# lebrice/blurred-GAN

Measured on AMD Instinct MI355X. Metric: images/sec (G+D+GP step), higher is better.
Workload: dtype f32; 1 GPU; celeba64 64x64x3 batch 256/GPU, blur sigma 5.0 (31 taps), D-step+GP+G-step+Adam; global_batch=256, parallelism=dp1

## Files before the change

blurred-gan_amd/csrc/conv_rows.hip:

```cpp
#include "conv_common.h"
#include <algorithm>
#include <cstdlib>
#include <cstring>
#include <type_traits>

namespace {

typedef float floatx4 __attribute__((ext_vector_type(4)));

struct RowParams {
  const float* A;
  const float* Wt;
  float* C;
  int B, Hi, Wi, Ck, Ho, Wo, N;
  int pt, pl, flip;
  int R, strips;
  int wpr, ipw;
  int epi_mode;
  const float* bias;
  const float* ref;
  const unsigned char* keep;
  size_t keep_elems;
  float alpha, scale;
};
// ... 82 lines not shown
  int e_src[NE][NTERM];
  unsigned e_dst[NE];
  float e_bias[NE], e_mul[NE];
  int e_n[NE];
  if (tid < 2 * S) pbuf[(size_t)tid * PS + PIXW * 17] = 0.f;
  {
    const int per_img = p.Wo * N;
#pragma unroll
    for (int q = 0; q < NE; ++q) {
      const int e = tid + q * NTH;
      const int im = e / per_img, rem = e - im * per_img;
      const int x = rem / N, n = rem - x * N;
      const bool ok = e < p.ipw * per_img && im < nimg;
      e_dst[q] = ok ? (unsigned)(((im * p.Ho * p.Wo + x) * N + n) * 4) : kOob;
      e_n[q] = n;
      e_bias[q] = ok && p.bias ? p.bias[n] : 0.f;
      e_mul[q] = ok && p.epi_mode == BG_EPI_AFFINE_LRELU ? p.ref[n] : 0.f;
#pragma unroll
      for (int i = 0; i < NTERM; ++i) {
        const int kw = (x + p.pl) % S + i * S;
        const int num = x + p.pl - kw, ix = num / S;
        e_src[q][i] = (ok && kw < K && num >= 0 && ix < p.Wi) ? (im * p.Wi + ix) * 17 + kw * N + n : PIXW * 17;
      }
    }
  }
  const size_t out0 = img0 * p.Ho * p.Wo * N;
  auto pwrite = [&](const floatx4& pacc, int slot) {
    float* pb = pbuf + (size_t)slot * PS;
#pragma unroll
    for (int rr = 0; rr < 4; ++rr) pb[((size_t)img * p.Wi + 16 * t + 4 * kq + rr) * 17 + li] = pacc[rr];
  };
  auto pstore = [&](int slot, int y, bool live) {
    const float* pb = pbuf + (size_t)slot * PS;
    float v[NE];
#pragma unroll
    for (int q = 0; q < NE; ++q) {
      v[q] = pb[e_src[q][0]];
#pragma unroll
      for (int i = 1; i < NTERM; ++i) v[q] += pb[e_src[q][i]];
    }
    const unsigned add = live ? (unsigned)(y * p.Wo * N * 4) : 0u, force = live ? 0u : kOob;
#pragma unroll
    for (int q = 0; q < NE; ++q) {
      const unsigned off = (e_dst[q] + add) | force;
      float o;
      if (EP == 0) {
        o = v[q] + e_bias[q];
      } else if (EP == 1) {
        o = tanh_branchless(v[q] + e_bias[q]);
      } else {
        const bool mine = (off & kOob) == 0;
        o = mine ? bg::apply_epilogue_pre(p, v[q], out0 + (off >> 2), e_bias[q], e_mul[q]) : 0.f;
      }
      __builtin_amdgcn_raw_buffer_store_b32(__builtin_bit_cast(unsigned, o), rsC, off, 0, 0);
    }
  };

  float4 g0[NQ], g1[NQ], g2[NQ], g3[NQ];
  gload(0, g0);
  gload(1, g1);
  gload(2, g2);
  gload(3, g3);
  lstore(0, g0);
  gload(4, g0);
#pragma unroll
  for (int i = 0; i < 4 * NE * S; ++i) __builtin_amdgcn_raw_buffer_store_b32(0u, rsC, kOob + 4u * i, 0, 0);
  int y_prev = 0;
  bool have_prev = false;
  auto flush_prev = [&](int prev_par) {
#pragma unroll
    for (int kh = 0; kh < S; ++kh) {
      const int y = y_prev + kh;
      pstore(prev_par * S + kh, y, have_prev & (y >= y0) & (y < y1));
    }
  };
  auto trip = [&](int r, auto parity, float4 (&g)[NQ]) {
    constexpr int cur = decltype(parity)::value;
    __syncthreads();
    float a[KS];
#pragma unroll
    for (int ks = 0; ks < KS; ++ks) a[ks] = afrag[(size_t)cur * PIXW * AS + 4 * ks];
#pragma unroll
    for (int ks = 0; ks < KS; ++ks)
#pragma unroll
      for (int kh = 0; kh < K; ++kh) acc[kh] = __builtin_amdgcn_mfma_f32_16x16x4f32(a[ks], bw[kh][ks], acc[kh], 0, 0, 0);
    flush_prev(cur ^ 1);
    lstore(cur ^ 1, g);
    gload(r + 5, g);
#pragma unroll
    for (int kh = 0; kh < S; ++kh) pwrite(acc[kh], cur * S + kh);
    y_prev = (iy_lo + r) * S - p.pt;
    have_prev = true;
#pragma unroll
    for (int i = 0; i < K; ++i) acc[i] = i + S < K ? acc[i + S] : floatx4{0.f, 0.f, 0.f, 0.f};
  };
  int r = 0;
  for (; r + 4 <= nrows; r += 4) {
    trip(r, std::integral_constant<int, 0>{}, g1);
    trip(r + 1, std::integral_constant<int, 1>{}, g2);
    trip(r + 2, std::integral_constant<int, 0>{}, g3);
    trip(r + 3, std::integral_constant<int, 1>{}, g0);
  }
  int last_par = 1;
  if (r < nrows) {
    trip(r, std::integral_constant<int, 0>{}, g1);
    last_par = 0;
    if (r + 1 < nrows) {
      trip(r + 1, std::integral_constant<int, 1>{}, g2);
      last_par = 1;
      if (r + 2 < nrows) {
        trip(r + 2, std::integral_constant<int, 0>{}, g3);
        last_par = 0;
      }
    }
  }
  __syncthreads();
  if (last_par == 0) flush_prev(0); else flush_prev(1);
}

template <int K, int S>
int launch_rows(const RowParams& p, dim3 grid, size_t lds, hipStream_t s) {
  const bool wide = p.Wi == 128;
  const int ep = p.epi_mode == BG_EPI_NONE ? 0 : p.epi_mode == BG_EPI_TANH ? 1 : 2;
#define BG_RS2(KSv, EPv) do { if (wide) bg::launch((conv_rows_scatter_kernel<KSv, K, S, 128, EPv>), grid, dim3(512), lds, s, p); \
                              else bg::launch((conv_rows_scatter_kernel<KSv, K, S, 64, EPv>), grid, dim3(256), lds, s, p); } while (0)
#define BG_RS(KSv) do { if (ep == 0) BG_RS2(KSv, 0); else if (ep == 1) BG_RS2(KSv, 1); else BG_RS2(KSv, 2); } while (0)
  switch (p.Ck) {
    case 16: BG_RS(4); return 1;
    case 32: BG_RS(8); return 1;
    case 64: BG_RS(16); return 1;
    default: return 0;
  }
#undef BG_RS
#undef BG_RS2
}

constexpr int kRgHalo = 16;

struct RowGParams {
  const float* A;
  const float* Wt;
  float* C;
  int B, Hi, Wi, Ct, Ho, Wo, N;
  int s, pt, pl, flip;
  int R, strips;
  int epi_mode;
  const float* bias;
  const float* ref;
  const unsigned char* keep;
  size_t keep_elems;
  float alpha, scale;
};

template <int TG, int NT, int K, bool MASK>
__global__ __launch_bounds__(256) void conv_rows_gather_kernel(const RowGParams p) {
  extern __shared__ __attribute__((aligned(16))) float xl[];
  const int tid = threadIdx.x, lane = tid & 63, wave = tid >> 6;
  const int li = lane & 15, kq = lane >> 4;
  const int Ct = p.Ct, N = 16 * NT, st = p.s;
  const int RS = p.Wi * Ct + 2 * kRgHalo;
  const int strip = blockIdx.x % p.strips, b = blockIdx.x / p.strips;
  const int oy0 = strip * p.R, rows = min(p.R, p.Ho - oy0);
  const int nrows_in = (rows - 1) * st + K;

  float bw[K][4][NT];
#pragma unroll
  for (int ks = 0; ks < 4; ++ks) {
    const int i = 4 * ks + kq, kw = i / Ct, ci = i - kw * Ct;
#pragma unroll
    for (int kh = 0; kh < K; ++kh) {
      const int tap = p.flip ? (K - 1 - kh) * K + (K - 1 - kw) : kh * K + kw;
#pragma unroll
      for (int nt = 0; nt < NT; ++nt) bw[kh][ks][nt] = i < K * Ct ? p.Wt[((size_t)tap * N + nt * 16 + li) * Ct + ci] : 0.f;
    }
  }
  const int RL = p.Wi * Ct;
  if ((RL & 3) == 0) {
    const int q4 = RS / 4;
    bg::stage_rows_f4<4>(xl, nrows_in, q4, RS, tid, [&](int r, int c4) -> const float* {
      const int iy = oy0 * st - p.pt + r, e = c4 * 4 - kRgHalo;
      return ((unsigned)iy < (unsigned)p.Hi && (unsigned)e < (unsigned)RL) ? p.A + ((size_t)b * p.Hi + iy) * RL + e : nullptr;
    });
  } else {
    for (int idx = tid; idx < nrows_in * RS; idx += 256) {
      const int r = idx / RS, c = idx - r * RS;
      const int iy = oy0 * st - p.pt + r, e = c - kRgHalo;
      float v = 0.f;
      if ((unsigned)iy < (unsigned)p.Hi && (unsigned)e < (unsigned)RL) v = p.A[((size_t)b * p.Hi + iy) * RL + e];
      xl[idx] = v;
    }
  }
  __syncthreads();

  float e_bias[NT], e_mul[NT];
#pragma unroll
  for (int nt = 0; nt < NT; ++nt) {
    e_bias[nt] = p.bias ? p.bias[nt * 16 + li] : 0.f;
    e_mul[nt] = p.epi_mode == BG_EPI_AFFINE_LRELU ? p.ref[nt * 16 + li] : 1.f;
  }
  const int groups = p.Wo / (16 * TG);
  const int nunits = rows * groups;
  for (int u = wave; u < nunits; u += 4) {
    const int r = u / groups, g = u - r * groups;
    const int oy = oy0 + r, ox0 = g * 16 * TG;
    floatx4 acc[TG][NT];
#pragma unroll
    for (int tg = 0; tg < TG; ++tg)
#pragma unroll
      for (int nt = 0; nt < NT; ++nt) acc[tg][nt] = floatx4{0.f, 0.f, 0.f, 0.f};
    const float* abase = xl + (size_t)(r * st) * RS + kRgHalo + ((ox0 + li) * st - p.pl) * Ct + kq;
#pragma unroll
    for (int kh = 0; kh < K; ++kh) {
      float a[TG][4];
#pragma unroll
      for (int tg = 0; tg < TG; ++tg)
#pragma unroll
        for (int ks = 0; ks < 4; ++ks) a[tg][ks] = abase[(size_t)kh * RS + tg * 16 * st * Ct + 4 * ks];
#pragma unroll
      for (int ks = 0; ks < 4; ++ks)
#pragma unroll
        for (int tg = 0; tg < TG; ++tg)
#pragma unroll
          for (int nt = 0; nt < NT; ++nt) acc[tg][nt] = __builtin_amdgcn_mfma_f32_16x16x4f32(a[tg][ks], bw[kh][ks][nt], acc[tg][nt], 0, 0, 0);
    }
    constexpr bool mask_epi = MASK;
#pragma unroll
    for (int tg = 0; tg < TG; ++tg) {
      const size_t pix0 = ((size_t)b * p.Ho + oy) * p.Wo + ox0 + 16 * tg + 4 * kq;
      unsigned char e_keep[4][NT];
      if (mask_epi) {
#pragma unroll
        for (int rr = 0; rr < 4; ++rr)
#pragma unroll
          for (int nt = 0; nt < NT; ++nt) {
            const size_t idx = (pix0 + rr) * N + nt * 16 + li;
            e_keep[rr][nt] = p.keep[(p.keep_elems == 0 || idx < p.keep_elems) ? idx : 0];
          }
      }
#pragma unroll
      for (int rr = 0; rr < 4; ++rr)
#pragma unroll
        for (int nt = 0; nt < NT; ++nt) {
          const size_t idx = (pix0 + rr) * N + nt * 16 + li;
          if (mask_epi) {
            float v = acc[tg][nt][rr] + e_bias[nt];
            v = v > 0.f ? v : p.alpha * v;
            if (p.keep_elems == 0 || idx < p.keep_elems) v = e_keep[rr][nt] ? v * p.scale : 0.f;
            p.C[idx] = v;
          } else {
            p.C[idx] = bg::apply_epilogue_pre(p, acc[tg][nt][rr], idx, e_bias[nt], e_mul[nt]);
          }
        }
    }
  }
}

template <int K>
int launch_rows_gather(const RowGParams& p, int tg, dim3 grid, size_t lds, hipStream_t s) {
  const int nt = p.N / 16;
  const bool mask = p.epi_mode == BG_EPI_BIAS_LRELU && p.keep != nullptr;
#define BG_RG(TGv, NTv) do { if (mask) bg::launch((conv_rows_gather_kernel<TGv, NTv, K, true>), grid, dim3(256), lds, s, p); \
                             else bg::launch((conv_rows_gather_kernel<TGv, NTv, K, false>), grid, dim3(256), lds, s, p); } while (0)
  if (tg == 1) { if (nt == 1) BG_RG(1, 1); else if (nt == 2) BG_RG(1, 2); else BG_RG(1, 4); }
  else if (tg == 2) { if (nt == 1) BG_RG(2, 1); else if (nt == 2) BG_RG(2, 2); else BG_RG(2, 4); }
  else { if (nt == 1) BG_RG(4, 1); else if (nt == 2) BG_RG(4, 2); else BG_RG(4, 4); }
#undef BG_RG
  return 1;
}

}

namespace bg {

int try_conv_rows_gather(int bwd_data, const float* a, const float* w, float* c, int B, int H, int W, int Cin, int Cout, int k, int s,
                         const bg_epilogue* epi, void* stream, int* taken) {
  *taken = 0;
  static const int off = getenv("BG_NO_ROWS") ? 1 : 0;
  if (off || (k != 5 && k != 3)) return BG_OK;
  RowGParams p;
  memset(&p, 0, sizeof p);
  int Ho, Wo, pt, pl;
  same_pads(H, k, s, &Ho, &pt);
  same_pads(W, k, s, &Wo, &pl);
  if (bwd_data) {
    if (s != 1 || Cout * k > 16 || (Cin != 16 && Cin != 32 && Cin != 64)) return BG_OK;
    p.Hi = H; p.Wi = W; p.Ct = Cout; p.Ho = H; p.Wo = W; p.N = Cin; p.s = 1; p.pt = k - 1 - pt; p.pl = k - 1 - pl; p.flip = 1;
  } else {
    if (Cin * k > 16 || (Cout != 16 && Cout != 32 && Cout != 64)) return BG_OK;
    p.Hi = H; p.Wi = W; p.Ct = Cin; p.Ho = Ho; p.Wo = Wo; p.N = Cout; p.s = s; p.pt = pt; p.pl = pl; p.flip = 0;
  }
  if (p.Wo % 16 != 0) return BG_OK;
  if ((size_t)B * p.Ho * p.Wo * p.N >= (1ull << 31)) return BG_OK;
  const int tiles = p.Wo / 16;
  const int tg = tiles % 4 == 0 ? 4 : (tiles % 2 == 0 ? 2 : 1);
  p.A = a; p.Wt = w; p.C = c; p.B = B;
  static const int rows_r = getenv("BG_ROWSG_R") ? atoi(getenv("BG_ROWSG_R")) : 0;
  p.R = std::min(rows_r ? rows_r : (s == 2 ? 8 : 16), p.Ho);
  p.strips = (int)cdiv(p.Ho, p.R);
  const size_t lds = ((size_t)((p.R - 1) * p.s + k) * (p.Wi * p.Ct + 2 * kRgHalo)) * sizeof(float);
  if (lds > 64 * 1024) return BG_OK;
  p.epi_mode = BG_EPI_NONE; p.alpha = 0.3f; p.scale = 1.f;
  if (epi) {
    BG_REQUIRE(epi->mode >= BG_EPI_NONE && epi->mode <= BG_EPI_AFFINE_LRELU, BG_ERR_UNSUPPORTED, "conv rows: epilogue mode %d", epi->mode);
    BG_REQUIRE(epi->mode != BG_EPI_MUL_GRAD || epi->ref, BG_ERR_NULL, "conv rows: BG_EPI_MUL_GRAD needs ref");
    BG_REQUIRE(epi->mode != BG_EPI_AFFINE_LRELU || (epi->ref && epi->bias), BG_ERR_NULL, "conv rows: BG_EPI_AFFINE_LRELU needs ref and bias");
    p.epi_mode = epi->mode; p.bias = epi->bias; p.ref = epi->ref; p.keep = epi->keep; p.keep_elems = epi->keep_elems; p.alpha = epi->alpha; p.scale = epi->scale;
  }
  const dim3 grid((unsigned)(B * p.strips));
  const double flops = 2.0 * B * (double)Ho * Wo * Cin * Cout * k * k;
  Launch L(stream, bwd_data ? "conv_rows_thin_k_dgrad" : "conv_rows_thin_k_fwd", flops, 0);
  if (k == 5) launch_rows_gather<5>(p, tg, grid, lds, L.s);
  else launch_rows_gather<3>(p, tg, grid, lds, L.s);
  *taken = 1;
  return L.done("conv_rows_gather_kernel");
}



int try_conv_rows(int bwd_data, const float* a, const float* w, float* c, int B, int H, int W, int Cin, int Cout, int k, int s,
                  const bg_epilogue* epi, void* stream, int* taken) {
  *taken = 0;
  static const int off = getenv("BG_NO_ROWS") ? 1 : 0;
  if (off || (k != 5 && k != 3)) return BG_OK;
  RowParams p;
  memset(&p, 0, sizeof p);
  int Ho, Wo, pt, pl;
  same_pads(H, k, s, &Ho, &pt);
  same_pads(W, k, s, &Wo, &pl);
  if (bwd_data) {
    if (Cin * k > 16 || (Cout != 16 && Cout != 32 && Cout != 64)) return BG_OK;
    p.Hi = Ho; p.Wi = Wo; p.Ck = Cout; p.Ho = H; p.Wo = W; p.N = Cin; p.pt = pt; p.pl = pl; p.flip = 0;
  } else {
    if (s != 1 || Cout * k > 16 || (Cin != 16 && Cin != 32 && Cin != 64)) return BG_OK;
    p.Hi = H; p.Wi = W; p.Ck = Cin; p.Ho = H; p.Wo = W; p.N = Cout; p.pt = k - 1 - pt; p.pl = k - 1 - pl; p.flip = 1;
  }
  if (p.Wi != 16 && p.Wi != 32 && p.Wi != 64 && p.Wi != 128) return BG_OK;
  if ((size_t)B * p.Hi * p.Wi * p.Ck >= (1ull << 31) || (size_t)B * p.Ho * p.Wo * p.N >= (1ull << 31)) return BG_OK;
  p.A = a; p.Wt = w; p.C = c; p.B = B;
  static const int rows_r = getenv("BG_ROWS_R") ? atoi(getenv("BG_ROWS_R")) : 0;
  p.R = std::min(rows_r ? rows_r : (s == 1 ? 32 : 16), p.Ho);
  p.strips = (int)cdiv(p.Ho, p.R);
  p.wpr = p.Wi / 16;
  p.ipw = p.Wi == 128 ? 1 : 4 / p.wpr;
  const int pixw = p.Wi == 128 ? 128 : 64;
  if ((long)p.ipw * p.Wo * p.N > (long)((s * (16 / k) + 3) / 4) * pixw * 4) return BG_OK;
  if ((size_t)p.ipw * p.Hi * p.Wi * p.Ck >= (1ull << 29) || (size_t)p.ipw * p.Ho * p.Wo * p.N >= (1ull << 29)) return BG_OK;
  p.epi_mode = BG_EPI_NONE; p.alpha = 0.3f; p.scale = 1.f;
  if (epi) {
    BG_REQUIRE(epi->mode >= BG_EPI_NONE && epi->mode <= BG_EPI_AFFINE_LRELU, BG_ERR_UNSUPPORTED, "conv rows: epilogue mode %d", epi->mode);
    BG_REQUIRE(epi->mode != BG_EPI_MUL_GRAD || epi->ref, BG_ERR_NULL, "conv rows: BG_EPI_MUL_GRAD needs ref");
    BG_REQUIRE(epi->mode != BG_EPI_AFFINE_LRELU || (epi->ref && epi->bias), BG_ERR_NULL, "conv rows: BG_EPI_AFFINE_LRELU needs ref and bias");
    p.epi_mode = epi->mode; p.bias = epi->bias; p.ref = epi->ref; p.keep = epi->keep; p.keep_elems = epi->keep_elems; p.alpha = epi->alpha; p.scale = epi->scale;
  }
  const dim3 grid((unsigned)(cdiv(B, p.ipw) * p.strips));
  const size_t lds = ((size_t)2 * pixw * (p.Ck + 4) + (size_t)2 * s * (pixw * 17 + 1)) * sizeof(float);
  const double flops = 2.0 * B * (double)H * W * Cin * Cout * k * k / (s * s);
  Launch L(stream, bwd_data ? "conv_rows_dgrad" : "conv_rows_fwd", flops, 0);
  int ok;
  if (k == 5) ok = s == 2 ? launch_rows<5, 2>(p, grid, lds, L.s) : launch_rows<5, 1>(p, grid, lds, L.s);
  else ok = s == 2 ? launch_rows<3, 2>(p, grid, lds, L.s) : launch_rows<3, 1>(p, grid, lds, L.s);
  (void)ok;
  *taken = 1;
  return L.done("conv_rows_scatter_kernel");
}

}
```

blurred-gan_amd/csrc/conv_wgrad.hip:

```cpp
#include "conv_common.h"
#include <algorithm>
#include <cmath>
#include <cstdlib>
#include <mutex>
#include <type_traits>
#include <utility>

namespace {

typedef float floatx16 __attribute__((ext_vector_type(16)));

struct WgradParams {
  const float* X;
  const float* DY;
  float* out;
  int B, H, W, Ci, Ho, Wo, Co;
  int k, s, pt, pl;
  int M;
  int chunk;
  int ksplit;
  int tiles_m, tiles_n, xcd_swizzle;
  float beta, scale;
  unsigned x_bytes, dy_bytes;
  unsigned mul_hw, sh_hw, mul_w, sh_w;
// ... 595 lines not shown
        }
      }
    }
    if (!A_IM2COL) {
#pragma unroll
      for (int i = 0; i < AP; ++i) {
        const int r = arow + i * RPP_A;
        if (r < BKP) *reinterpret_cast<float4*>(sa + r * BM + aq * 4) = regA[i];
      }
    }
    if (!B_IM2COL) {
#pragma unroll
      for (int i = 0; i < BP; ++i) {
        const int r = brow + i * RPP_B;
        if (r < BKP) *reinterpret_cast<float4*>(sb + r * BN + bq * 4) = regB[i];
      }
    }
  };

  floatx16 acc[MI][NI];
#pragma unroll
  for (int i = 0; i < MI; ++i)
#pragma unroll
    for (int j = 0; j < NI; ++j)
#pragma unroll
      for (int r = 0; r < 16; ++r) acc[i][j][r] = 0.f;

  if (nsteps > 0) {
    gload(0);
    lstore(0);
  }
  __syncthreads();
  const int fcol = lane & 31, fk = lane >> 5;
  for (int step = 0; step < nsteps; ++step) {
    const int cur = step & 1;
    if (step + 1 < nsteps) gload(step + 1);
    const float* sa = smem + cur * STAGE + wm * WTM + fcol;
    const float* sb = smem + cur * STAGE + BKP * BM + wn * WTN + fcol;
#pragma unroll 4
    for (int it = 0; it < BKP / 2 / WAVES_K; ++it) {
      const int krow = 2 * (wk + it * WAVES_K) + fk;
      float af[MI], bf[NI];
#pragma unroll
      for (int i = 0; i < MI; ++i) af[i] = sa[krow * BM + i * 32];
#pragma unroll
      for (int j = 0; j < NI; ++j) bf[j] = sb[krow * BN + j * 32];
#pragma unroll
      for (int i = 0; i < MI; ++i)
#pragma unroll
        for (int j = 0; j < NI; ++j) acc[i][j] = __builtin_amdgcn_mfma_f32_32x32x2f32(af[i], bf[j], acc[i][j], 0, 0, 0);
    }
    if (step + 1 < nsteps) lstore(cur ^ 1);
    __syncthreads();
  }

  if (WAVES_K > 1) {
    if (wk > 0) {
      float* red = smem + (((wk - 1) * WAVES_M * WAVES_N + wmn) * MI * NI) * 1024;
#pragma unroll
      for (int i = 0; i < MI; ++i)
#pragma unroll
        for (int j = 0; j < NI; ++j)
#pragma unroll
          for (int r = 0; r < 16; ++r) red[((i * NI + j) * 16 + r) * 64 + lane] = acc[i][j][r];
    }
    __syncthreads();
    if (wk > 0) return;
#pragma unroll
    for (int w = 1; w < WAVES_K; ++w) {
      const float* red = smem + (((w - 1) * WAVES_M * WAVES_N + wmn) * MI * NI) * 1024;
#pragma unroll
      for (int i = 0; i < MI; ++i)
#pragma unroll
        for (int j = 0; j < NI; ++j)
#pragma unroll
          for (int r = 0; r < 16; ++r) acc[i][j][r] += red[((i * NI + j) * 16 + r) * 64 + lane];
    }
  }

  const int kk = p.k * p.k;
  float* out = p.out + (size_t)blockIdx.z * kk * p.Ci * p.Co;
  const bool direct = p.ksplit == 1;
#pragma unroll
  for (int i = 0; i < MI; ++i)
#pragma unroll
    for (int j = 0; j < NI; ++j) {
      const int col = wn * WTN + j * 32 + (lane & 31);
#pragma unroll
      for (int r = 0; r < 16; ++r) {
        const int row = wm * WTM + i * 32 + (r & 3) + 8 * (r >> 2) + 4 * (lane >> 5);
        size_t idx;
        bool ok;
        if (MODE == 0) {
          const int ci = ci0 + row, co = co0 + col;
          ok = ci < p.Ci && co < p.Co;
          idx = ((size_t)tap * p.Ci + ci) * p.Co + co;
        } else if (MODE == 1) {
          const int co = co0 + col;
          ok = row < kk * p.Ci && co < p.Co;
          idx = (size_t)row * p.Co + co;
        } else {
          const int ci = ci0 + row;
          const int t = col / p.Co, co = col - t * p.Co;
          ok = ci < p.Ci && col < kk * p.Co;
          idx = ((size_t)t * p.Ci + ci) * p.Co + co;
        }
        if (ok) {
          float* q = out + idx;
          const float v = acc[i][j][r];
          if (direct) *q = (p.beta != 0.f ? p.beta * *q : 0.f) + p.scale * v;
          else *q = v;
        }
      }
    }
}

__global__ __launch_bounds__(256) void wgrad_direct_kernel(const WgradParams p) {
  const int nout = p.k * p.k * p.Ci * p.Co;
  const int e = blockIdx.x * 256 + threadIdx.x;
  if (e >= nout) return;
  const int co = e % p.Co;
  const int ci = (e / p.Co) % p.Ci;
  const int tap = e / (p.Co * p.Ci);
  const int kh = tap / p.k, kw = tap % p.k;
  const int m_begin = blockIdx.y * p.chunk, m_end = min(p.M, m_begin + p.chunk);
  const int HoWo = p.Ho * p.Wo;
  int b = m_begin / HoWo;
  int rem = m_begin - b * HoWo;
  int oh = rem / p.Wo, ow = rem - oh * p.Wo;
  float acc = 0.f;
  for (int m = m_begin; m < m_end; ++m) {
    const int iy = oh * p.s + kh - p.pt, ix = ow * p.s + kw - p.pl;
    if ((unsigned)iy < (unsigned)p.H && (unsigned)ix < (unsigned)p.W)
      acc = fmaf(p.X[((size_t)(b * p.H + iy) * p.W + ix) * p.Ci + ci], p.DY[(size_t)m * p.Co + co], acc);
    if (++ow == p.Wo) {
      ow = 0;
      if (++oh == p.Ho) { oh = 0; ++b; }
    }
  }
  float* q = p.out + (size_t)blockIdx.y * nout + e;
  if (p.ksplit == 1) *q = (p.beta != 0.f ? p.beta * *q : 0.f) + p.scale * acc;
  else *q = acc;
}

typedef float floatx4 __attribute__((ext_vector_type(4)));
constexpr int kTcRows = 16, kTcHalo = 8;

template <int MT, int K>
__global__ __launch_bounds__(256) void conv_wgrad_thin_co_kernel(const WgradParams p, int nblocks, int blocks_per_img) {
  extern __shared__ __attribute__((aligned(16))) float tc_lds[];
  const int W = p.W, H = p.H, Ci = 16 * MT, Co = p.Co;
  const int RS = W * Co + 2 * kTcHalo;
  const int nrows = kTcRows + K - 1;
  const int tid = threadIdx.x, lane = tid & 63, wave = tid >> 6;
  const int li = lane & 15, kq = lane >> 4;
  floatx4 acc[K][MT];
#pragma unroll
  for (int kh = 0; kh < K; ++kh)
#pragma unroll
    for (int mt = 0; mt < MT; ++mt) acc[kh][mt] = floatx4{0.f, 0.f, 0.f, 0.f};
  const int ncol = K * Co;
  const int kw_n = li / Co, co_n = li - kw_n * Co;
  const int b_base = li < ncol ? kTcHalo + (kq + p.pl - kw_n) * Co + co_n : 0;
  const int b_step = li < ncol ? 4 * Co : 0;
  const int ksteps = W / 4;

  for (int blk = blockIdx.x; blk < nblocks; blk += gridDim.x) {
    const int b = blk / blocks_per_img, y0 = (blk - b * blocks_per_img) * kTcRows;
    __syncthreads();
    if (((W * Co) & 3) == 0) {
      const int q4 = RS / 4;
      bg::stage_rows_f4<4>(tc_lds, nrows, q4, RS, tid, [&](int r, int c4) -> const float* {
        const int oy = y0 - (K - 1 - p.pt) + r, e = c4 * 4 - kTcHalo;
        return ((unsigned)oy < (unsigned)p.Ho && (unsigned)e < (unsigned)(W * Co)) ? p.DY + ((size_t)b * p.Ho + oy) * W * Co + e : nullptr;
      });
    } else {
      for (int idx = tid; idx < nrows * RS; idx += 256) {
        const int r = idx / RS, c = idx - r * RS;
        const int oy = y0 - (K - 1 - p.pt) + r, e = c - kTcHalo;
        float v = 0.f;
        if ((unsigned)oy < (unsigned)p.Ho && (unsigned)e < (unsigned)(W * Co)) v = p.DY[((size_t)b * p.Ho + oy) * W * Co + e];
        tc_lds[idx] = v;
      }
    }
    __syncthreads();
    const int groups = (ksteps + 7) / 8;
    const int myrows = min(kTcRows, H - y0);
    const int nitems = ((myrows - wave + 3) / 4) * groups;
    const float* xblk = p.X + ((size_t)b * H + y0) * W * Ci + kq * Ci + li;
    auto xload = [&](int it, float (&a)[8][MT]) {
      const int j = it / groups, g = it - j * groups;
      const float* xrow = xblk + (size_t)(wave + 4 * j) * W * Ci + (size_t)g * 32 * Ci;
#pragma unroll
      for (int q = 0; q < 8; ++q)
#pragma unroll
        for (int mt = 0; mt < MT; ++mt) a[q][mt] = (it < nitems && g * 8 + q < ksteps) ? xrow[(size_t)q * 4 * Ci + mt * 16] : 0.f;
    };
    auto compute = [&](int it, const float (&a)[8][MT]) {
      const int j = it / groups, g = it - j * groups;
      const int r = wave + 4 * j;
#pragma unroll
      for (int kh = 0; kh < K; ++kh) {
        const float* brow = tc_lds + (r + (K - 1) - kh) * RS + b_base + g * 8 * b_step;
#pragma unroll
        for (int q = 0; q < 8; ++q) {
          const float bv = brow[q * b_step];
#pragma unroll
          for (int mt = 0; mt < MT; ++mt) acc[kh][mt] = __builtin_amdgcn_mfma_f32_16x16x4f32(a[q][mt], bv, acc[kh][mt], 0, 0, 0);
        }
      }
    };
    float a0[8][MT], a1[8][MT];
    xload(0, a0);
    for (int it = 0; it < nitems; it += 2) {
      xload(it + 1, a1);
      compute(it, a0);
      xload(it + 2, a0);
      if (it + 1 < nitems) compute(it + 1, a1);
    }
  }
  __syncthreads();
  float* red = tc_lds;
#pragma unroll
  for (int kh = 0; kh < K; ++kh)
#pragma unroll
    for (int mt = 0; mt < MT; ++mt)
#pragma unroll
      for (int rr = 0; rr < 4; ++rr) red[((wave * K + kh) * MT * 4 + mt * 4 + rr) * 64 + lane] = acc[kh][mt][rr];
  __syncthreads();
  float* out = p.out + (size_t)blockIdx.x * K * K * Ci * Co;
  for (int e = tid; e < K * MT * 4 * 64; e += 256) {
    const int l = e & 63, slot = e >> 6;
    const int rr = slot & 3, mt = (slot >> 2) % MT, kh = slot / (4 * MT);
    const int n = l & 15;
    if (n >= ncol) continue;
    const float v = (red[(0 * K * MT * 4 + slot) * 64 + l] + red[(1 * K * MT * 4 + slot) * 64 + l]) +
                    (red[(2 * K * MT * 4 + slot) * 64 + l] + red[(3 * K * MT * 4 + slot) * 64 + l]);
    const int kw = n / Co, co = n - kw * Co, ci = mt * 16 + 4 * (l >> 4) + rr;
    out[((size_t)(kh * K + kw) * Ci + ci) * Co + co] = v;
  }
}

constexpr int kTiHalo = 16;

template <int NT, int K>
__global__ __launch_bounds__(256) void conv_wgrad_thin_ci_kernel(const WgradParams p, int nblocks, int blocks_per_img, int RB) {
  extern __shared__ __attribute__((aligned(16))) float ti_lds[];
  const int W = p.W, H = p.H, Ci = p.Ci, Co = 16 * NT, Ho = p.Ho, Wo = p.Wo, st = p.s;
  const int RS = W * Ci + 2 * kTiHalo;
  const int nrows = (RB - 1) * st + K;
  const int tid = threadIdx.x, lane = tid & 63, wave = tid >> 6;
  const int li = lane & 15, kq = lane >> 4;
  floatx4 acc[K][NT];
#pragma unroll
  for (int kh = 0; kh < K; ++kh)
#pragma unroll
    for (int nt = 0; nt < NT; ++nt) acc[kh][nt] = floatx4{0.f, 0.f, 0.f, 0.f};
  const int nrow_used = K * Ci;
  const int a_base = li < nrow_used ? kTiHalo + (kq * st - p.pl) * Ci + li : 0;
  const int a_step = li < nrow_used ? 4 * st * Ci : 0;
  const int ksteps = Wo / 4;
  const int groups = (ksteps + 7) / 8;

  for (int blk = blockIdx.x; blk < nblocks; blk += gridDim.x) {
    const int b = blk / blocks_per_img, oy0 = (blk - b * blocks_per_img) * RB;
    __syncthreads();
    if (((W * Ci) & 3) == 0) {
      const int q4 = RS / 4;
      bg::stage_rows_f4<4>(ti_lds, nrows, q4, RS, tid, [&](int r, int c4) -> const float* {
        const int yy = oy0 * st - p.pt + r, e = c4 * 4 - kTiHalo;
        return ((unsigned)yy < (unsigned)H && (unsigned)e < (unsigned)(W * Ci)) ? p.X + ((size_t)b * H + yy) * W * Ci + e : nullptr;
      });
    } else {
      for (int idx = tid; idx < nrows * RS; idx += 256) {
        const int r = idx / RS, c = idx - r * RS;
        const int yy = oy0 * st - p.pt + r, e = c - kTiHalo;
        float v = 0.f;
        if ((unsigned)yy < (unsigned)H && (unsigned)e < (unsigned)(W * Ci)) v = p.X[((size_t)b * H + yy) * W * Ci + e];
        ti_lds[idx] = v;
      }
    }
    __syncthreads();
    const int myrows = min(RB, Ho - oy0);
    const int nitems = ((myrows - wave + 3) / 4) * groups;
    const float* dyblk = p.DY + ((size_t)b * Ho + oy0) * Wo * Co + kq * Co + li;
    auto yload = [&](int it, float (&bv)[8][NT]) {
      const int j = it / groups, g = it - j * groups;
      const float* dyrow = dyblk + (size_t)(wave + 4 * j) * Wo * Co + (size_t)g * 32 * Co;
#pragma unroll
      for (int q = 0; q < 8; ++q)
#pragma unroll
        for (int nt = 0; nt < NT; ++nt) bv[q][nt] = (it < nitems && g * 8 + q < ksteps) ? dyrow[(size_t)q * 4 * Co + nt * 16] : 0.f;
    };
    auto compute = [&](int it, const float (&bv)[8][NT]) {
      const int j = it / groups, g = it - j * groups;
      const int r = wave + 4 * j;
#pragma unroll
      for (int kh = 0; kh < K; ++kh) {
        const float* arow = ti_lds + (r * st + kh) * RS + a_base + g * 8 * a_step;
#pragma unroll
        for (int q = 0; q < 8; ++q) {
          const float av = arow[q * a_step];
#pragma unroll
          for (int nt = 0; nt < NT; ++nt) acc[kh][nt] = __builtin_amdgcn_mfma_f32_16x16x4f32(av, bv[q][nt], acc[kh][nt], 0, 0, 0);
        }
      }
    };
    float b0[8][NT], b1[8][NT];
    yload(0, b0);
    for (int it = 0; it < nitems; it += 2) {
      yload(it + 1, b1);
      compute(it, b0);
      yload(it + 2, b0);
      if (it + 1 < nitems) compute(it + 1, b1);
    }
  }
  float* red = ti_lds;
  for (int w = 0; w < 4; ++w) {
    __syncthreads();
    if (wave == w) {
#pragma unroll
      for (int kh = 0; kh < K; ++kh)
#pragma unroll
        for (int nt = 0; nt < NT; ++nt)
#pragma unroll
          for (int rr = 0; rr < 4; ++rr) {
            float* q = red + ((kh * NT + nt) * 4 + rr) * 64 + lane;
            *q = (w == 0 ? 0.f : *q) + acc[kh][nt][rr];
          }
    }
  }
  __syncthreads();
  float* out = p.out + (size_t)blockIdx.x * K * K * Ci * Co;
  for (int e = tid; e < K * NT * 4 * 64; e += 256) {
    const int l = e & 63, slot = e >> 6;
    const int rr = slot & 3, nt = (slot >> 2) % NT, kh = slot / (4 * NT);
    const int i = 4 * (l >> 4) + rr;
    if (i >= nrow_used) continue;
    const int kw = i / Ci, ci = i - kw * Ci;
    out[((size_t)(kh * K + kw) * Ci + ci) * Co + nt * 16 + (l & 15)] = red[e];
  }
}

constexpr int kC16Rows = 7;

template <int WO>
__global__ __launch_bounds__(256) void conv_wgrad_c16_kernel(const WgradParams p, int nstrips, int strips_per_img) {
  constexpr int W = 2 * WO, PS = (WO + 2) * 16, RS = 2 * PS, KSW = WO / 8;
  constexpr int PFX = kC16Rows * W * 4 / 256;
  constexpr unsigned kOob = 0x80000000u;
  extern __shared__ __attribute__((aligned(16))) float c16_lds[];
  const int tid = threadIdx.x, lane = tid & 63, wave = tid >> 6;
  const int li = lane & 15, kq = lane >> 4;
  const int r = wave >> 1, half = wave & 1;
  const __amdgpu_buffer_rsrc_t rsX = __builtin_amdgcn_make_buffer_rsrc(const_cast<float*>(p.X), 0, (int)p.x_bytes, 0x00020000);
  const __amdgpu_buffer_rsrc_t rsY = __builtin_amdgcn_make_buffer_rsrc(const_cast<float*>(p.DY), 0, (int)p.dy_bytes, 0x00020000);

  for (int i = tid; i < 2 * kC16Rows * 2 * 2 * 16; i += 256) {
    const int e = i & 15, side = (i >> 4) & 1, plane = i >> 5;
    c16_lds[plane * PS + (side ? (WO + 1) * 16 : 0) + e] = 0.f;
  }
  floatx4 acc[25][2];
#pragma unroll
  for (int t = 0; t < 25; ++t) { acc[t][0] = floatx4{0.f, 0.f, 0.f, 0.f}; acc[t][1] = floatx4{0.f, 0.f, 0.f, 0.f}; }

  float4 pf[PFX];
  float bn[KSW][2], bc[KSW][2];
  auto prefetch = [&](int strip) {
    const int b = strip / strips_per_img, oy0 = (strip - b * strips_per_img) * 2;
    const bool live = strip < nstrips;
#pragma unroll
    for (int i = 0; i < PFX; ++i) {
      const int item = i * 256 + tid;
      const int rr = item / (W * 4), rem = item - rr * (W * 4);
      const int y = 2 * oy0 - 1 + rr;
      const bool ok = live && (unsigned)y < (unsigned)p.H;
      pf[i] = __builtin_bit_cast(float4, __builtin_amdgcn_raw_buffer_load_b128(rsX, ok ? (unsigned)(((b * p.H + y) * W) * 64 + rem * 16) : kOob, 0, 0));
    }
    const unsigned ybase = (unsigned)((((b * p.Ho + oy0 + r) * WO) + half * (WO / 2) + kq) * 128 + li * 4);
#pragma unroll
    for (int ks = 0; ks < KSW; ++ks)
#pragma unroll
      for (int nt = 0; nt < 2; ++nt)
        bn[ks][nt] = __builtin_bit_cast(float, __builtin_amdgcn_raw_buffer_load_b32(rsY, live ? ybase + (unsigned)(ks * 4 * 128 + nt * 64) : kOob, 0, 0));
  };
  auto stash = [&](int buf) {
    float* dst = c16_lds + buf * kC16Rows * RS;
#pragma unroll
    for (int i = 0; i < PFX; ++i) {
      const int item = i * 256 + tid;
      const int rr = item / (W * 4), rem = item - rr * (W * 4);
      const int x = rem >> 2, q = rem & 3;
      *reinterpret_cast<float4*>(dst + rr * RS + (x & 1) * PS + ((x >> 1) + 1) * 16 + q * 4) = pf[i];
    }
  };

  int strip = blockIdx.x;
  prefetch(strip);
  stash(0);
  __syncthreads();
  int buf = 0;
  for (; strip < nstrips; strip += gridDim.x, buf ^= 1) {
#pragma unroll
    for (int ks = 0; ks < KSW; ++ks) { bc[ks][0] = bn[ks][0]; bc[ks][1] = bn[ks][1]; }
    prefetch(strip + gridDim.x);
    const float* xb = c16_lds + buf * kC16Rows * RS + (2 * r) * RS + (half * (WO / 2) + kq + 1) * 16 + li;
#pragma unroll
    for (int ks = 0; ks < KSW; ++ks)
#pragma unroll
      for (int kh = 0; kh < 5; ++kh)
#pragma unroll
        for (int kw = 0; kw < 5; ++kw) {
          const int par = (kw + 1) & 1, fl = kw == 0 ? -1 : (kw - 1) / 2;
          const float a = xb[kh * RS + par * PS + (4 * ks + fl) * 16];
          acc[kh * 5 + kw][0] = __builtin_amdgcn_mfma_f32_16x16x4f32(a, bc[ks][0], acc[kh * 5 + kw][0], 0, 0, 0);
          acc[kh * 5 + kw][1] = __builtin_amdgcn_mfma_f32_16x16x4f32(a, bc[ks][1], acc[kh * 5 + kw][1], 0, 0, 0);
        }
    stash(buf ^ 1);
    __syncthreads();
  }
  float* red = c16_lds;
  for (int w = 0; w < 4; ++w) {
    __syncthreads();
    if (wave == w) {
#pragma unroll
      for (int t = 0; t < 25; ++t)
#pragma unroll
        for (int nt = 0; nt < 2; ++nt)
#pragma unroll
          for (int rr = 0; rr < 4; ++rr) {
            float* q = red + ((t * 2 + nt) * 4 + rr) * 64 + lane;
            *q = (w == 0 ? 0.f : *q) + acc[t][nt][rr];
          }
    }
  }
  __syncthreads();
  float* out = p.out + (size_t)blockIdx.x * 25 * 16 * 32;
  for (int e = tid; e < 25 * 2 * 4 * 64; e += 256) {
    const int l = e & 63, slot = e >> 6;
    const int rr = slot & 3, nt = (slot >> 2) & 1, t = slot >> 3;
    out[(size_t)(t * 16 + 4 * (l >> 4) + rr) * 32 + nt * 16 + (l & 15)] = red[e];
  }
}

template <int LGWO>
struct StripGeom {
  static constexpr int WO = 1 << LGWO, W = 2 * WO, R = 64 / WO, RX = 2 * R + 3, WP = W + 3;
  static constexpr int XROW = WP * 32, XBUF = RX * XROW, YBUF = 64 * 64, BUF = XBUF + YBUF;
  static constexpr int NX = RX * W * 8, NLX = (NX + 255) / 256, NL = NLX + 4;
  static constexpr size_t lds_bytes = (size_t)2 * BUF * sizeof(float);
};

typedef float floatx2 __attribute__((ext_vector_type(2)));

template <int O0>
__device__ inline void strip_read2(floatx2& dst, unsigned addr) {
  asm volatile("ds_read2st64_b32 %0, %1 offset0:%2 offset1:%3" : "=v"(dst) : "v"(addr), "n"(O0), "n"(O0 + 2));
}
__device__ inline void strip_mfma(floatx16& acc, float a, float b) {
  asm volatile("v_mfma_f32_32x32x2_f32 %0, %1, %2, %0" : "+a"(acc) : "v"(a), "v"(b));
}
template <int LGWO, int Q, int T>
__device__ inline void strip_fetch(floatx2 (&af)[13], floatx2& bf, const unsigned (&aaddr)[13], unsigned baddr) {
  constexpr int WO = 1 << LGWO, WP = 2 * WO + 3, pix = 4 * Q, oyl = pix >> LGWO, ox = pix & (WO - 1);
  if constexpr (T < 13) strip_read2<oyl * WP + ox>(af[T], aaddr[T]);
  else strip_read2<pix>(bf, baddr);
}
typedef float floatx4v __attribute__((ext_vector_type(4)));
__device__ inline void strip_gload(floatx4v& dst, unsigned off, __amdgpu_buffer_rsrc_t rs) {
// ... 620 lines not shown
```

Baseline: 32890 images/s.

## Use buffer loads/stores, uniform wave ids and specialized epilogues in row conv kernels

Rewrites the row-gather conv epilogue to use raw buffer stores and byte loads with per-image resource descriptors. It also specializes the epilogue mode and keep-mask coverage at compile time and replaces per-unit division with incremental row/group stepping. The wgrad kernels switch to buffer loads whose out-of-range reads return zero in place of branchy guarded loads, add sched barriers, and specialize constant strides (Co==3, st*Ci==6). The goal is less scalar/vector address arithmetic and fewer branches in hot loops, at the cost of more template instantiations and a new per-image size limit.

```diff
diff --git a/blurred-gan_amd/csrc/conv_rows.hip b/blurred-gan_amd/csrc/conv_rows.hip
--- a/blurred-gan_amd/csrc/conv_rows.hip
+++ b/blurred-gan_amd/csrc/conv_rows.hip
@@ -258,10 +258,31 @@
   float alpha, scale;
 };
 
+template <int MODE, bool KEEP, class P>
+__device__ inline float apply_epilogue_mode(const P& p, float v, size_t idx, float bias_n, float mul_n) {
+  if (MODE == BG_EPI_AFFINE_LRELU) {
+    v = fmaf(v, mul_n, bias_n);
+    return v > 0.f ? v : p.alpha * v;
+  }
+  v += bias_n;
+  if (MODE == BG_EPI_BIAS_LRELU) {
+    v = v > 0.f ? v : p.alpha * v;
+    if (KEEP && (p.keep_elems == 0 || idx < p.keep_elems)) v = p.keep[idx] ? v * p.scale : 0.f;
+  } else if (MODE == BG_EPI_MUL_GRAD) {
+    float f = p.ref[idx] > 0.f ? 1.f : p.alpha;
+    if (KEEP && (p.keep_elems == 0 || idx < p.keep_elems)) f = p.keep[idx] ? f * p.scale : 0.f;
+    v *= f;
+  } else if (MODE == BG_EPI_TANH) {
+    v = tanhf(v);
+  }
+  return v;
+}
+
 template <int TG, int NT, int K, bool MASK>
 __global__ __launch_bounds__(256) void conv_rows_gather_kernel(const RowGParams p) {
   extern __shared__ __attribute__((aligned(16))) float xl[];
-  const int tid = threadIdx.x, lane = tid & 63, wave = tid >> 6;
+  const int tid = threadIdx.x, lane = tid & 63;
+  const int wave = __builtin_amdgcn_readfirstlane(tid >> 6);
   const int li = lane & 15, kq = lane >> 4;
   const int Ct = p.Ct, N = 16 * NT, st = p.s;
   const int RS = p.Wi * Ct + 2 * kRgHalo;
@@ -306,22 +327,33 @@
   }
   const int groups = p.Wo / (16 * TG);
   const int nunits = rows * groups;
+  const int per_img = p.Ho * p.Wo * N;
+  const size_t img_e0 = (size_t)b * per_img;
+  const __amdgpu_buffer_rsrc_t rsC = __builtin_amdgcn_make_buffer_rsrc(p.C + img_e0, 0, per_img * 4, 0x00020000);
+  const unsigned lane_e = (unsigned)(4 * kq * N + li);
+  int cov = per_img;
+  if (MASK && p.keep_elems != 0) cov = p.keep_elems <= img_e0 ? 0 : (int)std::min<size_t>(p.keep_elems - img_e0, (size_t)per_img);
+  const __amdgpu_buffer_rsrc_t rsK =
+      __builtin_amdgcn_make_buffer_rsrc(const_cast<unsigned char*>(MASK ? p.keep + img_e0 : nullptr), 0, MASK ? cov : 0, 0x00020000);
+  const int a_lane = kRgHalo + (li * st - p.pl) * Ct + kq;
+  const int rstep = 4 / groups, gstep = 4 - rstep * groups;
+  auto units = [&](auto mode, auto keep, auto cover) {
+  int r = wave / groups, g = wave - r * groups;
   for (int u = wave; u < nunits; u += 4) {
-    const int r = u / groups, g = u - r * groups;
     const int oy = oy0 + r, ox0 = g * 16 * TG;
     floatx4 acc[TG][NT];
 #pragma unroll
     for (int tg = 0; tg < TG; ++tg)
 #pragma unroll
       for (int nt = 0; nt < NT; ++nt) acc[tg][nt] = floatx4{0.f, 0.f, 0.f, 0.f};
-    const float* abase = xl + (size_t)(r * st) * RS + kRgHalo + ((ox0 + li) * st - p.pl) * Ct + kq;
+    const float* abase = xl + ((r * st) * RS + ox0 * st * Ct) + a_lane;
 #pragma unroll
     for (int kh = 0; kh < K; ++kh) {
       float a[TG][4];
 #pragma unroll
       for (int tg = 0; tg < TG; ++tg)
 #pragma unroll
-        for (int ks = 0; ks < 4; ++ks) a[tg][ks] = abase[(size_t)kh * RS + tg * 16 * st * Ct + 4 * ks];
+        for (int ks = 0; ks < 4; ++ks) a[tg][ks] = abase[kh * RS + tg * 16 * st * Ct + 4 * ks];
 #pragma unroll
       for (int ks = 0; ks < 4; ++ks)
 #pragma unroll
@@ -329,35 +361,71 @@
 #pragma unroll
           for (int nt = 0; nt < NT; ++nt) acc[tg][nt] = __builtin_amdgcn_mfma_f32_16x16x4f32(a[tg][ks], bw[kh][ks][nt], acc[tg][nt], 0, 0, 0);
     }
-    constexpr bool mask_epi = MASK;
+    const int unit_e = (oy * p.Wo + ox0) * N;
 #pragma unroll
     for (int tg = 0; tg < TG; ++tg) {
-      const size_t pix0 = ((size_t)b * p.Ho + oy) * p.Wo + ox0 + 16 * tg + 4 * kq;
-      unsigned char e_keep[4][NT];
-      if (mask_epi) {
+      const int tile_e = unit_e + tg * 16 * N;
+      if (MASK) {
+        constexpr int CV = decltype(cover)::value;
+        const int left = cov - tile_e;
+        unsigned char e_keep[4][NT];
+        if (CV != 0) {
+#pragma unroll
+          for (int rr = 0; rr < 4; ++rr)
+#pragma unroll
+            for (int nt = 0; nt < NT; ++nt)
+              e_keep[rr][nt] = __builtin_amdgcn_raw_buffer_load_b8(rsK, lane_e + (unsigned)(rr * N + nt * 16), tile_e, 0);
+        }
 #pragma unroll
         for (int rr = 0; rr < 4; ++rr)
 #pragma unroll
           for (int nt = 0; nt < NT; ++nt) {
-            const size_t idx = (pix0 + rr) * N + nt * 16 + li;
-            e_keep[rr][nt] = p.keep[(p.keep_elems == 0 || idx < p.keep_elems) ? idx : 0];
+            const unsigned e = lane_e + (unsigned)(rr * N + nt * 16);
+            float v = acc[tg][nt][rr] + e_bias[nt];
+            v = v > 0.f ? v : p.alpha * v;
+            if (CV == 1 || (CV == 2 && (int)e < left)) v = e_keep[rr][nt] ? v * p.scale : 0.f;
+            __builtin_amdgcn_raw_buffer_store_b32(__builtin_bit_cast(unsigned, v), rsC, e * 4u, tile_e * 4, 0);
+          }
+      } else {
+#pragma unroll
+        for (int rr = 0; rr < 4; ++rr)
+#pragma unroll
+          for (int nt = 0; nt < NT; ++nt) {
+            const unsigned e = lane_e + (unsigned)(rr * N + nt * 16);
+            const float v = apply_epilogue_mode<decltype(mode)::value, decltype(keep)::value>(p, acc[tg][nt][rr], img_e0 + (size_t)tile_e + e,
+                                                                                                  e_bias[nt], e_mul[nt]);
+            __builtin_amdgcn_raw_buffer_store_b32(__builtin_bit_cast(unsigned, v), rsC, e * 4u, tile_e * 4, 0);
           }
       }
-#pragma unroll
-      for (int rr = 0; rr < 4; ++rr)
-#pragma unroll
-        for (int nt = 0; nt < NT; ++nt) {
-          const size_t idx = (pix0 + rr) * N + nt * 16 + li;
-          if (mask_epi) {
-            float v = acc[tg][nt][rr] + e_bias[nt];
-            v = v > 0.f ? v : p.alpha * v;
-            if (p.keep_elems == 0 || idx < p.keep_elems) v = e_keep[rr][nt] ? v * p.scale : 0.f;
-            p.C[idx] = v;
-          } else {
-            p.C[idx] = bg::apply_epilogue_pre(p, acc[tg][nt][rr], idx, e_bias[nt], e_mul[nt]);
-          }
-        }
-    }
+    }
+    r += rstep;
+    g += gstep;
+    if (g >= groups) {
+      g -= groups;
+      ++r;
+    }
+  }
+  };
+  using std::integral_constant;
+  const integral_constant<int, 0> c0{};
+  if (MASK) {
+    if (cov == per_img) units(integral_constant<int, BG_EPI_BIAS_LRELU>{}, std::true_type{}, integral_constant<int, 1>{});
+    else if (cov == 0) units(integral_constant<int, BG_EPI_BIAS_LRELU>{}, std::true_type{}, c0);
+    else units(integral_constant<int, BG_EPI_BIAS_LRELU>{}, std::true_type{}, integral_constant<int, 2>{});
+    return;
+  }
+  switch (p.epi_mode) {
+    case BG_EPI_AFFINE_LRELU: units(integral_constant<int, BG_EPI_AFFINE_LRELU>{}, std::false_type{}, c0); break;
+    case BG_EPI_BIAS_LRELU:
+      if (p.keep) units(integral_constant<int, BG_EPI_BIAS_LRELU>{}, std::true_type{}, c0);
+      else units(integral_constant<int, BG_EPI_BIAS_LRELU>{}, std::false_type{}, c0);
+      break;
+    case BG_EPI_MUL_GRAD:
+      if (p.keep) units(integral_constant<int, BG_EPI_MUL_GRAD>{}, std::true_type{}, c0);
+      else units(integral_constant<int, BG_EPI_MUL_GRAD>{}, std::false_type{}, c0);
+      break;
+    case BG_EPI_TANH: units(integral_constant<int, BG_EPI_TANH>{}, std::false_type{}, c0); break;
+    default: units(integral_constant<int, BG_EPI_NONE>{}, std::false_type{}, c0); break;
   }
 }
 
@@ -397,6 +465,7 @@
   }
   if (p.Wo % 16 != 0) return BG_OK;
   if ((size_t)B * p.Ho * p.Wo * p.N >= (1ull << 31)) return BG_OK;
+  if ((size_t)p.Ho * p.Wo * p.N >= (1ull << 29)) return BG_OK;
   const int tiles = p.Wo / 16;
   const int tg = tiles % 4 == 0 ? 4 : (tiles % 2 == 0 ? 2 : 1);
   p.A = a; p.Wt = w; p.C = c; p.B = B;
diff --git a/blurred-gan_amd/csrc/conv_wgrad.hip b/blurred-gan_amd/csrc/conv_wgrad.hip
--- a/blurred-gan_amd/csrc/conv_wgrad.hip
+++ b/blurred-gan_amd/csrc/conv_wgrad.hip
@@ -771,7 +771,7 @@
   const int W = p.W, H = p.H, Ci = 16 * MT, Co = p.Co;
   const int RS = W * Co + 2 * kTcHalo;
   const int nrows = kTcRows + K - 1;
-  const int tid = threadIdx.x, lane = tid & 63, wave = tid >> 6;
+  const int tid = threadIdx.x, lane = tid & 63, wave = __builtin_amdgcn_readfirstlane(tid >> 6);
   const int li = lane & 15, kq = lane >> 4;
   floatx4 acc[K][MT];
 #pragma unroll
@@ -781,9 +781,11 @@
   const int ncol = K * Co;
   const int kw_n = li / Co, co_n = li - kw_n * Co;
   const int b_base = li < ncol ? kTcHalo + (kq + p.pl - kw_n) * Co + co_n : 0;
-  const int b_step = li < ncol ? 4 * Co : 0;
   const int ksteps = W / 4;
 
+  auto blocks = [&](auto cco) {
+  constexpr int kCo = decltype(cco)::value;
+  const int b_step = 4 * (kCo ? kCo : Co);
   for (int blk = blockIdx.x; blk < nblocks; blk += gridDim.x) {
     const int b = blk / blocks_per_img, y0 = (blk - b * blocks_per_img) * kTcRows;
     __syncthreads();
@@ -806,17 +808,20 @@
     const int groups = (ksteps + 7) / 8;
     const int myrows = min(kTcRows, H - y0);
     const int nitems = ((myrows - wave + 3) / 4) * groups;
-    const float* xblk = p.X + ((size_t)b * H + y0) * W * Ci + kq * Ci + li;
-    auto xload = [&](int it, float (&a)[8][MT]) {
-      const int j = it / groups, g = it - j * groups;
-      const float* xrow = xblk + (size_t)(wave + 4 * j) * W * Ci + (size_t)g * 32 * Ci;
+    const float* xblk = p.X + ((size_t)b * H + y0) * W * Ci;
+    const unsigned x_lane = (unsigned)((kq * Ci + li) * 4);
+    auto xload = [&](int it, int j, int g, float (&a)[8][MT]) {
+      const bool live = it < nitems;
+      const __amdgpu_buffer_rsrc_t rs = __builtin_amdgcn_make_buffer_rsrc(const_cast<float*>(xblk + (size_t)(live ? wave + 4 * j : 0) * W * Ci), 0,
+                                                                           live ? W * Ci * 4 : 0, 0x00020000);
+      const int soff = live ? g * 32 * Ci * 4 : 0;
 #pragma unroll
       for (int q = 0; q < 8; ++q)
 #pragma unroll
-        for (int mt = 0; mt < MT; ++mt) a[q][mt] = (it < nitems && g * 8 + q < ksteps) ? xrow[(size_t)q * 4 * Ci + mt * 16] : 0.f;
+        for (int mt = 0; mt < MT; ++mt)
+          a[q][mt] = __builtin_bit_cast(float, __builtin_amdgcn_raw_buffer_load_b32(rs, x_lane + (unsigned)((q * 4 * Ci + mt * 16) * 4), soff, 0));
     };
-    auto compute = [&](int it, const float (&a)[8][MT]) {
-      const int j = it / groups, g = it - j * groups;
+    auto compute = [&](int j, int g, const float (&a)[8][MT]) {
       const int r = wave + 4 * j;
 #pragma unroll
       for (int kh = 0; kh < K; ++kh) {
@@ -829,15 +834,34 @@
         }
       }
     };
+    auto next_item = [&](int& j, int& g) {
+      if (++g == groups) {
+        g = 0;
+        ++j;
+      }
+    };
     float a0[8][MT], a1[8][MT];
-    xload(0, a0);
+    int j0 = 0, g0 = 0;
+    xload(0, j0, g0, a0);
     for (int it = 0; it < nitems; it += 2) {
-      xload(it + 1, a1);
-      compute(it, a0);
-      xload(it + 2, a0);
-      if (it + 1 < nitems) compute(it + 1, a1);
-    }
-  }
+      int j1 = j0, g1 = g0;
+      next_item(j1, g1);
+      int j2 = j1, g2 = g1;
+      next_item(j2, g2);
+      xload(it + 1, j1, g1, a1);
+      __builtin_amdgcn_sched_barrier(0);
+      compute(j0, g0, a0);
+      __builtin_amdgcn_sched_barrier(0);
+      xload(it + 2, j2, g2, a0);
+      __builtin_amdgcn_sched_barrier(0);
+      if (it + 1 < nitems) compute(j1, g1, a1);
+      j0 = j2;
+      g0 = g2;
+    }
+  }
+  };
+  if (Co == 3) blocks(std::integral_constant<int, 3>{});
+  else blocks(std::integral_constant<int, 0>{});
   __syncthreads();
   float* red = tc_lds;
 #pragma unroll
@@ -868,7 +892,7 @@
   const int W = p.W, H = p.H, Ci = p.Ci, Co = 16 * NT, Ho = p.Ho, Wo = p.Wo, st = p.s;
   const int RS = W * Ci + 2 * kTiHalo;
   const int nrows = (RB - 1) * st + K;
-  const int tid = threadIdx.x, lane = tid & 63, wave = tid >> 6;
+  const int tid = threadIdx.x, lane = tid & 63, wave = __builtin_amdgcn_readfirstlane(tid >> 6);
   const int li = lane & 15, kq = lane >> 4;
   floatx4 acc[K][NT];
 #pragma unroll
@@ -877,10 +901,12 @@
     for (int nt = 0; nt < NT; ++nt) acc[kh][nt] = floatx4{0.f, 0.f, 0.f, 0.f};
   const int nrow_used = K * Ci;
   const int a_base = li < nrow_used ? kTiHalo + (kq * st - p.pl) * Ci + li : 0;
-  const int a_step = li < nrow_used ? 4 * st * Ci : 0;
   const int ksteps = Wo / 4;
   const int groups = (ksteps + 7) / 8;
 
+  auto blocks = [&](auto csc) {
+  constexpr int kSC = decltype(csc)::value;
+  const int a_step = 4 * (kSC ? kSC : st * Ci);
   for (int blk = blockIdx.x; blk < nblocks; blk += gridDim.x) {
     const int b = blk / blocks_per_img, oy0 = (blk - b * blocks_per_img) * RB;
     __syncthreads();
@@ -902,17 +928,20 @@
     __syncthreads();
     const int myrows = min(RB, Ho - oy0);
     const int nitems = ((myrows - wave + 3) / 4) * groups;
-    const float* dyblk = p.DY + ((size_t)b * Ho + oy0) * Wo * Co + kq * Co + li;
-    auto yload = [&](int it, float (&bv)[8][NT]) {
-      const int j = it / groups, g = it - j * groups;
-      const float* dyrow = dyblk + (size_t)(wave + 4 * j) * Wo * Co + (size_t)g * 32 * Co;
+    const float* dyblk = p.DY + ((size_t)b * Ho + oy0) * Wo * Co;
+    const unsigned y_lane = (unsigned)((kq * Co + li) * 4);
+    auto yload = [&](int it, int j, int g, float (&bv)[8][NT]) {
+      const bool live = it < nitems;
+      const __amdgpu_buffer_rsrc_t rs = __builtin_amdgcn_make_buffer_rsrc(const_cast<float*>(dyblk + (size_t)(live ? wave + 4 * j : 0) * Wo * Co), 0,
+                                                                           live ? Wo * Co * 4 : 0, 0x00020000);
+      const int soff = live ? g * 32 * Co * 4 : 0;
 #pragma unroll
       for (int q = 0; q < 8; ++q)
 #pragma unroll
-        for (int nt = 0; nt < NT; ++nt) bv[q][nt] = (it < nitems && g * 8 + q < ksteps) ? dyrow[(size_t)q * 4 * Co + nt * 16] : 0.f;
+        for (int nt = 0; nt < NT; ++nt)
+          bv[q][nt] = __builtin_bit_cast(float, __builtin_amdgcn_raw_buffer_load_b32(rs, y_lane + (unsigned)((q * 4 * Co + nt * 16) * 4), soff, 0));
     };
-    auto compute = [&](int it, const float (&bv)[8][NT]) {
-      const int j = it / groups, g = it - j * groups;
+    auto compute = [&](int j, int g, const float (&bv)[8][NT]) {
       const int r = wave + 4 * j;
 #pragma unroll
       for (int kh = 0; kh < K; ++kh) {
@@ -925,15 +954,34 @@
         }
       }
     };
+    auto next_item = [&](int& j, int& g) {
+      if (++g == groups) {
+        g = 0;
+        ++j;
+      }
+    };
     float b0[8][NT], b1[8][NT];
-    yload(0, b0);
+    int j0 = 0, g0 = 0;
+    yload(0, j0, g0, b0);
     for (int it = 0; it < nitems; it += 2) {
-      yload(it + 1, b1);
-      compute(it, b0);
-      yload(it + 2, b0);
-      if (it + 1 < nitems) compute(it + 1, b1);
-    }
-  }
+      int j1 = j0, g1 = g0;
+      next_item(j1, g1);
+      int j2 = j1, g2 = g1;
+      next_item(j2, g2);
+      yload(it + 1, j1, g1, b1);
+      __builtin_amdgcn_sched_barrier(0);
+      compute(j0, g0, b0);
+      __builtin_amdgcn_sched_barrier(0);
+      yload(it + 2, j2, g2, b0);
+      __builtin_amdgcn_sched_barrier(0);
+      if (it + 1 < nitems) compute(j1, g1, b1);
+      j0 = j2;
+      g0 = g2;
+    }
+  }
+  };
+  if (st * Ci == 6) blocks(std::integral_constant<int, 6>{});
+  else blocks(std::integral_constant<int, 0>{});
   float* red = ti_lds;
   for (int w = 0; w < 4; ++w) {
     __syncthreads();
```

Result: no change. 33090 images/s, median of 6 (+0.6%).
